# fxcawley/nanoSandbox

Hardware: AMD Instinct MI355X
Metric: tokens/sec (whole node) GPT-2 124M DDP (higher is better)
Workload: dtype bf16

## Files before the change

csrc/kernels/gemm_wg4.hip:

```cpp
#include <utility>

#include "common.h"

namespace {

constexpr int W_BM = 256, W_BN = 256, W_BK = 64;
constexpr int W_THR = 256;
constexpr int W_IMG = W_BK * 256 * 2;
constexpr int W_SMEM = 4 * W_IMG;
constexpr int W_GRP = 3072;

enum : int { W_EPI_ATOMIC = 1, W_EPI_STORE = 4 };

typedef int w_i32x4 __attribute__((ext_vector_type(4)));

struct Wg4Args {
  const bf16_t* A;
  const bf16_t* B;
  float* C;
  float* gb;
  int M, N, K;
  int lda, ldb, ldc;
  int tiles_m, tiles_n, splits;
};

template <int I>
struct WI {
  static constexpr int value = I;
};
template <class F, int... Is>
__device__ __forceinline__ void w_for_impl(F&& f, std::integer_sequence<int, Is...>) {
  (f(WI<Is>{}), ...);
}
template <int N, class F>
__device__ __forceinline__ void w_for(F&& f) {
  w_for_impl(f, std::make_integer_sequence<int, N>{});
}

template <bool H>
__device__ __forceinline__ void w_mfma(f32x4& acc, const bf16x8& b, const bf16x8& a) {
  if constexpr (H) asm volatile("v_mfma_f32_16x16x32_f16 %0, %1, %2, %0" : "+a"(acc) : "v"(b), "v"(a));
  else asm volatile("v_mfma_f32_16x16x32_bf16 %0, %1, %2, %0" : "+a"(acc) : "v"(b), "v"(a));
}
// ... 14 lines not shown
}
template <int OFF>
__device__ __forceinline__ void w_dma(uint32_t lds, uint32_t voff, w_i32x4 rsrc, uint32_t soff) {
  if constexpr (OFF == 0) {
    asm volatile("s_mov_b32 m0, %0\n\ts_nop 0\n\tbuffer_load_dwordx4 %1, %2, %3 offen lds" ::"s"(lds), "v"(voff),
                 "s"(rsrc), "s"(soff)
                 : "memory");
  } else {
    asm volatile("buffer_load_dwordx4 %0, %1, %2 offen offset:%3 lds" ::"v"(voff), "s"(rsrc), "s"(soff), "n"(OFF)
                 : "memory");
  }
}
#ifndef NSA_WG4_GLDS
#define NSA_WG4_GLDS 0
#endif
template <int OFF>
__device__ __forceinline__ void w_dmag(uint32_t lds, uint32_t voff, const void* sbase) {
  if constexpr (OFF == 0) {
    asm volatile("s_mov_b32 m0, %0\n\ts_nop 0\n\tglobal_load_lds_dwordx4 %1, %2" ::"s"(lds), "v"(voff), "s"(sbase)
                 : "memory");
  } else {
    asm volatile("global_load_lds_dwordx4 %0, %1 offset:%2" ::"v"(voff), "s"(sbase), "n"(OFF) : "memory");
  }
}
__device__ __forceinline__ w_i32x4 w_rsrc(const void* base, uint32_t bytes) {
  const uint64_t b = (uint64_t)(uintptr_t)base;
  w_i32x4 r;
  r.x = __builtin_amdgcn_readfirstlane((int)(uint32_t)b);
  r.y = __builtin_amdgcn_readfirstlane((int)(uint32_t)(b >> 32) & 0xffff);
  r.z = __builtin_amdgcn_readfirstlane((int)bytes);
  r.w = 0x00020000;
  return r;
}
__device__ __forceinline__ void w_add_base(w_i32x4& r, uint32_t bytes) {
  uint64_t b = ((uint64_t)(uint32_t)r.y << 32) | (uint32_t)r.x;
  b += bytes;
  r.x = (int)(uint32_t)b;
  r.y = (int)(uint32_t)(b >> 32);
}
__device__ __forceinline__ s16x4 w_tr(uint32_t addr) {
  return __builtin_amdgcn_ds_read_tr16_b64_v4i16((__attribute__((address_space(3))) s16x4*)(uintptr_t)addr);
}
__device__ __forceinline__ bf16x8 w_cat(s16x4 a, s16x4 b) {
  typedef short s16x8 __attribute__((ext_vector_type(8)));
  s16x8 v = __builtin_shufflevector(a, b, 0, 1, 2, 3, 4, 5, 6, 7);
  return __builtin_bit_cast(bf16x8, v);
// ... 93 lines not shown
      w_dmag<(p & 3) * 1024>(dmaA + buf + (uint32_t)((p & 4) * 1024), vpA[p], sbase(ra));
    else
      w_dma<(p & 3) * 1024>(dmaA + buf + (uint32_t)((p & 4) * 1024), voA[(p & 1) | ((p >> 2) << 1)], ra, soA[p]);
  };
  auto issue_b = [&](uint32_t buf, auto P) {
    constexpr int p = decltype(P)::value;
    if constexpr (NSA_WG4_GLDS)
      w_dmag<(p & 3) * 1024>(dmaB + buf + (uint32_t)((p & 4) * 1024), vpB[p], sbase(rb));
    else
      w_dma<(p & 3) * 1024>(dmaB + buf + (uint32_t)((p & 4) * 1024), voB[(p & 1) | ((p >> 2) << 1)], rb, soB[p]);
  };

  const int ig = lane & 15, fq = ig >> 2, fp = ig & 3;
  const int krow = 8 * (lane >> 4) + fq;
  const int gk = w_g(krow);
  uint32_t rdA[8], rdB[8];
#pragma unroll
  for (int f = 0; f < 8; ++f) {
    const int fa = wm * 8 + f, fb = wn * 8 + f;
    rdA[f] = lds0 + (uint32_t)(krow * 512 + (((2 * fa + (fp >> 1)) ^ (2 * gk)) << 4) + (fp & 1) * 8);
    rdB[f] = lds0 + (uint32_t)(2 * W_IMG + krow * 512 + (((2 * fb + (fp >> 1)) ^ (2 * gk)) << 4) + (fp & 1) * 8);
  }

  w_for<8>([&](auto P) { issue_a(0, P); });
  w_for<8>([&](auto P) { issue_b(0, P); });
  cur_next();
  w_for<8>([&](auto P) { issue_a(W_IMG, P); });
  w_for<8>([&](auto P) { issue_b(W_IMG, P); });
  w_vmwait<16>();
  cur_next();
  w_barrier();

  f32x4 acc[8][8];
  bf16x8 a0[8], b0[8], a1[8], b1[8];
#pragma unroll
  for (int f = 0; f < 8; ++f) {
    a0[f] = w_cat(w_tr(rdA[f]), w_tr(rdA[f] + 2048));
    b0[f] = w_cat(w_tr(rdB[f]), w_tr(rdB[f] + 2048));
  }

  float bsum[8] = {0.f, 0.f, 0.f, 0.f, 0.f, 0.f, 0.f, 0.f};
  int kc = kt0;
  uint32_t buf = 0;
  auto ktile = [&](auto FIRST_) {
    constexpr bool FIRST = decltype(FIRST_)::value;
    const bool do_bg = BG && kc % g.tiles_n == tn;
    w_for<128>([&](auto I) {
      constexpr int n = decltype(I)::value;
      constexpr int kk = n >> 6, j = (n >> 3) & 7, i = n & 7;
      if constexpr (kk == 0) {
        if constexpr (FIRST) w_mfma0<H>(acc[i][j], b0[j], a0[i]);
        else w_mfma<H>(acc[i][j], b0[j], a0[i]);
      } else {
        w_mfma<H>(acc[i][j], b1[j], a1[i]);
      }
      if constexpr (BG && j == 1) {
// ... 14 lines not shown
        constexpr int pc = (n - D0) / DS;
        if constexpr (pc < 8) issue_a(buf, WI<pc>{});
        else issue_b(buf, WI<pc - 8>{});
      }
      if constexpr (n == 62) {
#pragma unroll
        for (int f = 0; f < 8; ++f) {
          rdA[f] ^= (uint32_t)W_IMG;
          rdB[f] ^= (uint32_t)W_IMG;
        }
      }
      if constexpr (n == 92) w_vmwait<(92 - D0) / DS + 1>();
      if constexpr (n == 93) w_barrier();
      if constexpr (n >= 94 && n < 126 && ((n - 94) & 1) == 0) {
        constexpr int f = ((n - 94) >> 1) & 7;
        if constexpr (n < 110) b0[f] = w_cat(w_tr(rdB[f]), w_tr(rdB[f] + 2048));
        else a0[f] = w_cat(w_tr(rdA[f]), w_tr(rdA[f] + 2048));
      }
    });
    buf ^= (uint32_t)W_IMG;
    cur_next();
    ++kc;
  };
  ktile(WI<1>{});
  for (int kt = 1; kt < nk; ++kt) ktile(WI<0>{});
  asm volatile("s_waitcnt vmcnt(0) lgkmcnt(0)\n\ts_nop 7\n\ts_nop 7\n\ts_nop 7" ::: "memory");
  if constexpr (BG) {
    const int first = kt0 + ((tn - kt0 % g.tiles_n) + g.tiles_n) % g.tiles_n;
    if (first < kt1) {
#pragma unroll
      for (int f = 0; f < 8; ++f) {
        if ((f & 1) != wn) continue;
        float v = bsum[f];
        v += __shfl_xor(v, 16);
        v += __shfl_xor(v, 32);
        const int m = m0 + wm * 128 + 16 * f + (lane & 15);
        if (lane < 16 && m >= mlo) atomicAdd(g.gb + m, v);
      }
    }
  }
  w_barrier();

  char* ep = smem + wave * 32768;
  const int er = lane & 15, eq = lane >> 4;
  float* Cz = g.C;
  if constexpr (EPI == W_EPI_STORE) Cz += (int64_t)z * g.M * g.ldc;
#pragma unroll
  for (int half = 0; half < 2; ++half) {
#pragma unroll
    for (int ii = 0; ii < 4; ++ii) {
      const int i = 4 * half + ii;
      const int row = 16 * ii + er;
#pragma unroll
      for (int j = 0; j < 8; ++j) {
        const int u = 4 * j + eq;
        *reinterpret_cast<f32x4*>(ep + row * 512 + ((u ^ (row & 7)) << 4)) = acc[i][j];
      }
    }
    __builtin_amdgcn_fence(__ATOMIC_SEQ_CST, "wavefront");
    __builtin_amdgcn_wave_barrier();
    const int col0 = n0 + wn * 128;
    const int rot = (z * 23) & 63;
#pragma unroll 4
    for (int r2 = 0; r2 < 64; ++r2) {
      const int rr = (r2 + rot) & 63;
      const int grow = m0 + wm * 128 + 64 * half + rr;
#pragma unroll
      for (int c2 = 0; c2 < 2; ++c2) {
        const int c = 64 * c2 + lane;
        const float val = *reinterpret_cast<const float*>(ep + rr * 512 + ((((c >> 2) ^ (rr & 7))) << 4) + (c & 3) * 4);
        if (grow >= mlo && col0 + c >= nlo) {
          if constexpr (EPI == W_EPI_STORE)
            Cz[(int64_t)grow * g.ldc + col0 + c] = val;
          else
            atomicAdd(Cz + (int64_t)grow * g.ldc + col0 + c, val);
        }
      }
    }
    __builtin_amdgcn_fence(__ATOMIC_SEQ_CST, "wavefront");
    __builtin_amdgcn_wave_barrier();
  }
}

namespace {
template <bool H>
hipError_t wgrad4_entry(int epi, const void* A, int lda, const void* B, int ldb, void* C, int ldc, void* gb, int M,
                        int N, int K, int splits, hipStream_t s) {
  if (gb && epi != W_EPI_ATOMIC) return hipErrorInvalidValue;
  if ((epi != W_EPI_ATOMIC && epi != W_EPI_STORE) || M < W_BM || N < W_BN || M % 8 || N % 8 || K % W_BK ||
      splits < 1 || splits > K / W_BK || lda % 8 || ldb % 8 || lda < M || ldb < N || ldc < N)
    return hipErrorInvalidValue;
  if ((int64_t)W_BK * lda * 2 + W_GRP >= (1ll << 31) || (int64_t)W_BK * ldb * 2 + W_GRP >= (1ll << 31))
    return hipErrorInvalidValue;
  Wg4Args a{};
  a.A = (const bf16_t*)A;
  a.B = (const bf16_t*)B;
  a.C = (float*)C;
  a.M = M;
  a.N = N;
  a.K = K;
  a.lda = lda;
  a.ldb = ldb;
  a.ldc = ldc;
  a.tiles_m = (M + W_BM - 1) / W_BM;
  a.tiles_n = (N + W_BN - 1) / W_BN;
  a.splits = splits;
  const dim3 grid(a.tiles_m * a.tiles_n * splits);
  a.gb = (float*)gb;
  if (gb) wgrad4_kernel<W_EPI_ATOMIC, true, H><<<grid, W_THR, 0, s>>>(a);
  else if (epi == W_EPI_ATOMIC) wgrad4_kernel<W_EPI_ATOMIC, false, H><<<grid, W_THR, 0, s>>>(a);
  else wgrad4_kernel<W_EPI_STORE, false, H><<<grid, W_THR, 0, s>>>(a);
  return hipGetLastError();
}
}

NSA_API hipError_t nsa_gemm_wgrad4b(int epi, const void* A, int lda, const void* B, int ldb, void* C, int ldc, void* gb,
                                    int M, int N, int K, int splits, hipStream_t s) {
  return wgrad4_entry<false>(epi, A, lda, B, ldb, C, ldc, gb, M, N, K, splits, s);
}
NSA_API hipError_t nsa_gemm_wgrad4(int epi, const void* A, int lda, const void* B, int ldb, void* C, int ldc, int M,
                                   int N, int K, int splits, hipStream_t s) {
  return wgrad4_entry<false>(epi, A, lda, B, ldb, C, ldc, nullptr, M, N, K, splits, s);
}
NSA_API hipError_t nsa_gemm_wgrad4b_h(int epi, const void* A, int lda, const void* B, int ldb, void* C, int ldc,
                                      void* gb, int M, int N, int K, int splits, hipStream_t s) {
  return wgrad4_entry<true>(epi, A, lda, B, ldb, C, ldc, gb, M, N, K, splits, s);
}
NSA_API hipError_t nsa_gemm_wgrad4_h(int epi, const void* A, int lda, const void* B, int ldb, void* C, int ldc, int M,
                                     int N, int K, int splits, hipStream_t s) {
  return wgrad4_entry<true>(epi, A, lda, B, ldb, C, ldc, nullptr, M, N, K, splits, s);
}
```

nanosandbox_amd/ops/_lib.py:

```python

from __future__ import annotations

import ctypes
import os
import threading

import torch

_LIB_DIR = os.path.join(os.path.dirname(os.path.dirname(os.path.abspath(__file__))), "lib")
LIB_PATH = os.environ.get("NSA_KERNEL_LIB") or os.path.join(_LIB_DIR, "libnsa_kernels.so")

_lock = threading.Lock()
_lib = None

c_void_p = ctypes.c_void_p
c_int = ctypes.c_int
c_int64 = ctypes.c_int64
c_uint64 = ctypes.c_uint64
c_float = ctypes.c_float

_SIGNATURES = {
    "nsa_embedding_fwd": [c_void_p, c_void_p, c_void_p, c_void_p, c_int, c_int, c_int, c_float, c_uint64, c_void_p],
    "nsa_embedding_bwd": [c_void_p, c_void_p, c_void_p, c_void_p, c_int, c_int, c_int, c_float, c_uint64, c_void_p],
    "nsa_embedding_fwd_x32": [c_void_p, c_void_p, c_void_p, c_void_p, c_int, c_int, c_int, c_float, c_uint64,
# ... 55 lines not shown
                           c_void_p],
    "nsa_skinny_ln_gemm_q8": [c_void_p, c_void_p, c_void_p, c_void_p, c_void_p, c_float, c_void_p, c_void_p,
                              c_void_p, c_void_p, c_int, c_int, c_int, c_int, c_int, c_void_p],
    "nsa_gemv_emb_ln_q8": [c_void_p, c_void_p, c_void_p, c_void_p, c_void_p, c_void_p, c_void_p, c_void_p, c_void_p,
                           c_void_p, c_void_p, c_int, c_int, c_float, c_int, c_int, c_void_p],
    "nsa_gemv_attn_q8": [c_void_p, c_int, c_void_p, c_void_p, c_void_p, c_void_p, c_int, c_int, c_int, c_int,
                         c_void_p],
    "nsa_gemv_ln_q8": [c_void_p, c_void_p, c_void_p, c_void_p, c_void_p, c_void_p, c_void_p, c_void_p, c_void_p,
                       c_int, c_int, c_float, c_int, c_int, c_void_p, c_void_p],
    "nsa_flash_bwd2": [c_void_p, c_void_p, c_void_p, c_void_p, c_void_p, c_void_p,
                       c_int, c_int, c_int, c_int, c_float, c_float, c_uint64, c_void_p],
    "nsa_rng_advance": [c_void_p],
    "nsa_rng_set": [c_uint64, c_void_p],
    "nsa_splitk_reduce": [c_void_p, c_void_p, c_int64, c_int, c_void_p],
    "nsa_embedding_bwd_det": [c_void_p, c_void_p, c_void_p, c_void_p, c_void_p, c_void_p, c_void_p, c_int, c_int,
                              c_int, c_int, c_int, c_float, c_uint64, c_void_p],
    "nsa_transpose_bf16": [c_void_p, c_void_p, c_int, c_int, c_void_p],
    "nsa_gemm": [c_int, c_int, c_void_p, c_int, c_void_p, c_int, c_void_p, c_int, c_void_p, c_void_p,
                 c_int, c_int, c_int, c_int, c_void_p],
    "nsa_gemm_wgrad4": [c_int, c_void_p, c_int, c_void_p, c_int, c_void_p, c_int, c_int, c_int, c_int, c_int,
                        c_void_p],
    "nsa_gemm_wgrad4b": [c_int, c_void_p, c_int, c_void_p, c_int, c_void_p, c_int, c_void_p, c_int, c_int, c_int, c_int,
                         c_void_p],
    "nsa_gemm_nt4": [c_int, c_void_p, c_int, c_void_p, c_int, c_void_p, c_int, c_void_p, c_void_p, c_void_p,
                     c_int, c_int, c_int, c_int, c_void_p],
    "nsa_gemm_small": [c_int, c_void_p, c_int, c_void_p, c_int, c_void_p, c_int, c_void_p, c_void_p, c_void_p,
                       c_int, c_int, c_int, c_void_p],
    "nsa_gemm_nt4_xent": [c_void_p, c_int, c_void_p, c_int, c_void_p, c_int, c_void_p, c_void_p, c_int, c_int, c_int,
                          c_int, c_int, c_void_p],
    "nsa_gemm_nt4_xdx": [c_void_p, c_int, c_void_p, c_int, c_void_p, c_int, c_void_p, c_void_p, c_int, c_int, c_int,
                         c_int, c_void_p],
    "nsa_xent_tlogit": [c_void_p, c_int, c_void_p, c_int, c_void_p, c_void_p, c_void_p, c_int, c_int, c_int, c_float,
                        c_void_p],
    "nsa_xent_combine": [c_void_p, c_int, c_void_p, c_void_p, c_void_p, c_void_p, c_void_p, c_int, c_float, c_float,
                         c_float, c_void_p],
    "nsa_xent_fixup": [c_void_p, c_int, c_void_p, c_int, c_void_p, c_int, c_void_p, c_void_p, c_void_p, c_void_p,
                       c_void_p, c_int, c_int, c_int, c_void_p],
    "nsa_xent_bwd_prep": [c_void_p, c_int, c_void_p, c_int, c_void_p, c_void_p, c_void_p, c_void_p, c_void_p,
                          c_void_p, c_int, c_int, c_void_p],
    "nsa_xent_dw_fix": [c_void_p, c_int, c_void_p, c_int, c_void_p, c_void_p, c_void_p, c_void_p, c_int, c_int, c_int,
                        c_void_p],
    "nsa_xent_dw_fix_sorted": [c_void_p, c_int, c_void_p, c_int, c_void_p, c_void_p, c_void_p, c_void_p, c_void_p,
                               c_void_p, c_void_p, c_void_p, c_int, c_int, c_int, c_int, c_void_p],
    "nsa_embedding_bwd_lds": [c_void_p, c_void_p, c_void_p, c_void_p, c_void_p, c_int, c_int, c_int, c_int, c_int,
                              c_float, c_uint64, c_void_p],
    "nsa_seg_lds_parts": [c_int],
    "nsa_xent_dw_fix_lds": [c_void_p, c_int, c_void_p, c_int, c_void_p, c_void_p, c_void_p, c_void_p, c_void_p,
                            c_int, c_int, c_int, c_int, c_void_p],
    "nsa_colsum_bf16_partial": [c_void_p, c_int, c_int, c_int, c_void_p, c_int, c_void_p],
    "nsa_keysort": [c_void_p, c_int, c_int, c_int, c_void_p, c_void_p, c_void_p, c_void_p, c_void_p],
    "nsa_keysort_ws_bytes": [c_int],
    "nsa_probe_spin": [c_int, c_uint64, c_void_p, c_void_p],
    "nsa_probe_mark": [c_void_p, c_void_p],
}
_RESTYPES = {"nsa_keysort_ws_bytes": c_int64}


class KernelLibraryMissing(RuntimeError):
    pass


def lib():
    global _lib
    if _lib is not None:
        return _lib
    with _lock:
        if _lib is not None:
            return _lib
        if not os.path.exists(LIB_PATH):
            raise KernelLibraryMissing(
                f"HIP kernel library not found at {LIB_PATH}; build it with "
                "`python -m nanosandbox_amd.build` (hipcc --offload-arch=gfx950)")
        L = ctypes.CDLL(LIB_PATH, mode=ctypes.RTLD_GLOBAL)
        for name, argtypes in _SIGNATURES.items():
            for sym in (name, name + "_h"):
                fn = getattr(L, sym, None)
                if fn is None:
                    continue
# ... 33 lines not shown
```

nanosandbox_amd/ops/gemm.py:

```python

from __future__ import annotations

import os

import torch

from . import _lib

BF16 = torch.bfloat16
F16 = torch.float16
LAYOUT_TN = 2


def _sym(name, t):
    if t.dtype == F16:
        return name + "_h"
    if t.dtype != BF16:
        raise ValueError(f"GEMM kernels take bf16 or fp16 operands, got {t.dtype}")
    return name
EPI_ATOMIC, EPI_STORE_F32 = 1, 4
BK = 64
TILE = 256


def _check(t, name):
# ... 199 lines not shown
                      _lib.ptr(g32), K_in, _lib.ptr(gb32), N_out, K_in, T, splits, _lib.stream())
            return g32
        wgrad_acc(dy2, x2, g32, splits, deterministic)
        bias_grad_acc(dy2, gb32, deterministic)
        return g32

    def launch(epi, C):
        if four:
            _lib.call(_sym("nsa_gemm_wgrad4", dy2), epi, _lib.ptr(dy2), dy2.stride(0), _lib.ptr(x2), x2.stride(0), _lib.ptr(C),
                      K_in, N_out, K_in, T, splits, _lib.stream())
        else:
            _lib.call(_sym("nsa_gemm", dy2), LAYOUT_TN, epi, _lib.ptr(dy2), dy2.stride(0), _lib.ptr(x2), x2.stride(0),
                      _lib.ptr(C), K_in, None, None, N_out, K_in, T, splits, _lib.stream())

    if deterministic and splits > 1:
        ws = torch.empty(splits, N_out, K_in, device=g32.device, dtype=torch.float32)
        launch(EPI_STORE_F32, ws)
        _lib.call("nsa_splitk_reduce", _lib.ptr(ws), _lib.ptr(g32), g32.numel(), splits, _lib.stream())
        return g32
    launch(EPI_ATOMIC, g32)
    return g32


def bias_grad_acc(dy2, gb32, deterministic=False):
    T, N = dy2.shape
    _check(dy2, "dy")
    nblk = max(1, min(256, T // 64))
    part = torch.empty(nblk, N, device=dy2.device, dtype=torch.float32)
    _lib.call(_sym("nsa_colsum_bf16_partial", dy2), _lib.ptr(dy2), dy2.stride(0), T, N, _lib.ptr(part), nblk, _lib.stream())
    _lib.call("nsa_colsum_accum_ordered" if deterministic else "nsa_colsum_accum", _lib.ptr(part), _lib.ptr(gb32),
              nblk, N, _lib.stream())
    return gb32
```

nanosandbox_amd/ops/gemm_dispatch.py:

```python

from __future__ import annotations

import os

import torch

from . import _lib
from . import gemm as _gemm

F32 = torch.float32
BF16 = torch.bfloat16

DETERMINISTIC = False


F16 = torch.float16



def _ok(*ts):
    return (ts[0].dtype in (BF16, F16)
            and all(t.is_cuda and t.dtype == ts[0].dtype and t.is_contiguous() and t.data_ptr() % 16 == 0
                    for t in ts))


def kernel_for(op: str, M: int, N: int, K: int) -> str:
# ... 41 lines not shown


def _gelu_grad_torch(uf):
    cdf = 0.5 * (1.0 + torch.erf(uf * 0.7071067811865476))
    return cdf + uf * torch.exp(-0.5 * uf * uf) * 0.3989422804014327


def fwd(x2, w, b=None):
    return _nt(x2, w, bias=b)


def fwd_gelu(x2, w, b=None):
    return _nt(x2, w, epi=_gemm.NT_EPI_GELU, bias=b, op="fwd_gelu")


def dgrad(dy2, w):
    return _nt(dy2, _wt(w), op="dgrad")


def dgrad_dgelu(dy2, w, gp):
    return _nt(dy2, _wt(w), epi=_gemm.NT_EPI_DGELU, u=gp, op="dgrad_dgelu")


def wgrad_acc(dy2, x2, g32, gb32=None):
    T, N = dy2.shape
    K = x2.shape[1]
    k = kernel_for("wgrad", N, K, T) if _ok(dy2, x2) and g32.is_contiguous() else "torch"
    _used.setdefault(("wgrad", N, K, T), k if k == "torch" else f"{k}/s{_gemm.wgrad_splits(N, K, T)}")
    if k != "torch":
        if gb32 is not None and not (gb32.is_contiguous() and dy2.shape[1] % 8 == 0):
            _gemm.wgrad_acc(dy2, x2, g32, deterministic=DETERMINISTIC)
            bias_grad_acc(dy2, gb32)
            return
        _gemm.wgrad_acc(dy2, x2, g32, deterministic=DETERMINISTIC, gb32=gb32)
        return
    g32.add_(dy2.t().float() @ x2.float())
    if gb32 is not None:
        gb32.add_(dy2.float().sum(0))


def bias_grad_acc(dy2, gb32):
    if _ok(dy2) and dy2.shape[1] % 8 == 0 and gb32.is_contiguous():
        _gemm.bias_grad_acc(dy2, gb32, deterministic=DETERMINISTIC)
        return
    gb32.add_(dy2.float().sum(0))


_weight_gen = 0


def weights_changed():
# ... 28 lines not shown
```

nanosandbox_amd/optim/flat.py:

```python

from __future__ import annotations

from dataclasses import dataclass

import torch

CHUNK = 64


@dataclass
class ParamSlot:
    name: str
    param: torch.nn.Parameter
    offset: int
    numel: int
    padded: int
    decay: bool


class FlatParamStore:
    def __init__(self, model: torch.nn.Module, device, compute_dtype=None, fused_grad=True):
        self.device = torch.device(device)
        named = [(n, p) for n, p in model.named_parameters() if p.requires_grad]
        self.slots: list[ParamSlot] = []
        off = 0
        for name, p in reversed(named):
            n = p.numel()
            rows = getattr(p, "_nsa_pad_rows", None)
            room = rows * p.shape[1] if rows and p.dim() == 2 and rows > p.shape[0] else n
            padded = (room + CHUNK - 1) // CHUNK * CHUNK
            self.slots.append(ParamSlot(name, p, off, n, padded, p.dim() >= 2))
            off += padded
        self.numel = off
        self.master = torch.zeros(off, dtype=torch.float32, device=self.device)
        self.grad = torch.zeros(off, dtype=torch.float32, device=self.device)
        flags = torch.zeros(off // CHUNK, dtype=torch.uint8)
        with torch.no_grad():
            for s in self.slots:
                view = self.master[s.offset:s.offset + s.numel]
                view.copy_(s.param.detach().reshape(-1).to(self.device, torch.float32))
                s.param.data = view.view(s.param.shape)
                if s.decay:
                    flags[s.offset // CHUNK:(s.offset + s.padded) // CHUNK] = 1
        self.wd_mask = flags.to(self.device)
        self.fused_grad = fused_grad
        for s in self.slots:
            g = self.grad[s.offset:s.offset + s.numel].view(s.param.shape)
            if fused_grad:
                s.param.main_grad = g
                pr = self._pad_shape(s)
                if pr is not None:
                    s.param.main_grad_padded = self.grad[s.offset:s.offset + pr[0] * pr[1]].view(pr)
            else:
                s.param.grad = g
        self.compute_dtype = compute_dtype
        self.compute = None
        if compute_dtype is not None and compute_dtype != torch.float32:
            self.compute = torch.empty(off, dtype=compute_dtype, device=self.device)
            for s in self.slots:
                s.param.compute = self.compute[s.offset:s.offset + s.numel].view(s.param.shape)
                pr = self._pad_shape(s)
                if pr is not None:
                    s.param.compute_padded = self.compute[s.offset:s.offset + pr[0] * pr[1]].view(pr)
            self.refresh_compute()

    @staticmethod
    def _pad_shape(s: ParamSlot):
        rows = getattr(s.param, "_nsa_pad_rows", None)
# ... 4 lines not shown
    def slot_of(self, p) -> ParamSlot:
        for s in self.slots:
            if s.param is p:
                return s
        raise KeyError("parameter not in store")

    def param_view(self, buf: torch.Tensor, s: ParamSlot) -> torch.Tensor:
        return buf[s.offset:s.offset + s.numel].view(s.param.shape)

    @torch.no_grad()
    def refresh_compute(self):
        from ..ops import gemm_dispatch
        gemm_dispatch.weights_changed()
        if self.compute is None:
            return
        if self.device.type == "cuda":
            from ..ops import _lib
            name = "nsa_cast_f32_bf16_h" if self.compute.dtype == torch.float16 else "nsa_cast_f32_bf16"
            _lib.call(name, _lib.ptr(self.master), _lib.ptr(self.compute), self.numel, _lib.stream())
        else:
            self.compute.copy_(self.master)

    @torch.no_grad()
    def zero_grad(self):
        self.grad.zero_()
        if not self.fused_grad:
            for s in self.slots:
                if s.param.grad is None or s.param.grad.data_ptr() != self.param_view(self.grad, s).data_ptr():
                    s.param.grad = self.param_view(self.grad, s)

    def buckets(self, cap_bytes: int):
        out = []
        start = 0
        size = 0
        members = []
        late = False
        for s in self.slots:
            nbytes = s.padded * 4
            is_late = bool(getattr(s.param, "_nsa_late_grad", False))
            if members and (is_late != late or (size + nbytes > cap_bytes and not is_late)):
                out.append((start, s.offset, members))
                start = s.offset
                size = 0
                members = []
            members.append(s)
            size += nbytes
            late = is_late
        if members:
# ... 3 lines not shown
```

nanosandbox_amd/runtime/hipgraph.py:

```python

from __future__ import annotations

import torch


def graph_capture_supported(device: str, dropout: float, world_size: int, ddp_impl: str = "flat",
                            gas: int = 2) -> tuple[bool, str]:
    if not str(device).startswith("cuda") or not torch.cuda.is_available():
        return False, "graph capture needs a GPU device"
    if world_size > 1 and ddp_impl != "flat":
        return False, "torch DDP: its reducer hooks autograd (use ddp_impl='flat')"
    if world_size > 1 and gas < 2:
        return False, "one micro-step per rank: the synchronising micro-step always runs eagerly"
    return True, ""


class MicroStepGraph:

    def __init__(self, model, X: torch.Tensor, Y: torch.Tensor, gas: int, warmup: int = 2, zero_grad=None,
                 dropout: bool = False, loss_scale: torch.Tensor | None = None):
        from ..ops import rng_advance

        self.model = model
        self.gas = gas
        self.X = X.detach().clone()
        self.Y = Y.detach().clone()
        side = torch.cuda.Stream()
        side.wait_stream(torch.cuda.current_stream())
        with torch.cuda.stream(side):
            for _ in range(warmup):
                if dropout:
                    rng_advance(self.X.device)
                _, loss = model(self.X, self.Y)
                ((loss / gas) * loss_scale if loss_scale is not None else loss / gas).backward()
        torch.cuda.current_stream().wait_stream(side)
        torch.cuda.synchronize()
        if zero_grad is not None:
            zero_grad()
        self.graph = torch.cuda.CUDAGraph()
        with torch.cuda.graph(self.graph):
            if dropout:
                rng_advance(self.X.device)
            _, loss = model(self.X, self.Y)
            self.loss = loss / gas
            (self.loss * loss_scale if loss_scale is not None else self.loss).backward()
        self.replays = 0

    def run(self, X: torch.Tensor, Y: torch.Tensor) -> torch.Tensor:
        self.X.copy_(X, non_blocking=True)
        self.Y.copy_(Y, non_blocking=True)
        self.graph.replay()
        self.replays += 1
        return self.loss
```

nanosandbox_amd/train.py:

```python

from __future__ import annotations

import os
import sys
import time

import torch

from .config import TRAIN_DEFAULTS, config_keys, parse_argv
from .data import load_meta, make_batch_source, resolve_data_dir
from .ops import rng_advance
from .ops.functional import XENT_F16_GUARD as xent_f16_guard
from .runtime import MicroStepGraph, graph_capture_supported
from .models import GPT, GPTConfig
from .optim import FlatParamStore
from .parallel import FlatBucketReducer, destroy, init_distributed
from .utils import MetricsLogger, get_lr, load_checkpoint, load_model_state, save_checkpoint


_DTYPES = {"bfloat16": torch.bfloat16, "float16": torch.float16, "float32": torch.float32}


def _compute_dtype(device_type: str, dtype: str) -> torch.dtype:
    if dtype not in _DTYPES:
        raise ValueError(f"dtype must be one of {sorted(_DTYPES)}, got {dtype!r}")
    if device_type != "cuda":
        return torch.float32
    return _DTYPES[dtype]


class Trainer:
    def __init__(self, cfg: dict):
        self.cfg = cfg
        c = cfg
        self.info = init_distributed(c["backend"], c["device"])
# ... 79 lines not shown
        fused_grad = self.ddp_impl != "torch"
        shadow = self.compute_dtype if self.compute_dtype in (torch.bfloat16, torch.float16) else None
        self.store = FlatParamStore(model, self.device, compute_dtype=shadow if self.device_type == "cuda" else None,
                                    fused_grad=fused_grad)
        self.optimizer = model.configure_optimizers(c["weight_decay"], c["learning_rate"], (c["beta1"], c["beta2"]),
                                                    self.device_type, store=self.store)
        if self.scaler is not None:
            self.optimizer.attach_loss_scale(self.scaler)
        if init_from == "resume" and checkpoint is not None:
            self.optimizer.load_state_dict(checkpoint["optimizer"])
        checkpoint = None
        self.activation_plan = None
        if self.device_type == "cuda" and (c["grad_ckpt"] or c["hbm_plan"]):
            from .utils.memory import plan_grad_ckpt
            free, _ = torch.cuda.mem_get_info(torch.device(self.device))
            self.activation_plan = plan_grad_ckpt(
                model.config.n_layer, model.config.n_embd, model.config.n_head, model.config.vocab_size,
                c["batch_size"] * c["block_size"], free, fp32_residual=c["fp32_residual"], requested=c["grad_ckpt"],
                recompute_mlp=c["recompute_mlp"])
            model.grad_ckpt = self.activation_plan.grad_ckpt
            model.recompute_mlp = self.activation_plan.recompute_mlp
            if self.master:
                print(self.activation_plan.describe())
        self.graph = None
        self.use_graph = False
        if c["compile"]:
            ok, why = graph_capture_supported(self.device, c["dropout"], info.world_size, self.ddp_impl, self.gas)
            if ok and self.compute_dtype not in (torch.bfloat16, torch.float16):
                ok, why = False, f"dtype={c['dtype']} runs the torch reference ops"
            self.use_graph = ok
            if self.master:
                print(("compile=True: micro-step captured as a HIP graph" +
                       (" (the synchronising micro-step runs eagerly)" if info.world_size > 1 else "")) if ok
                      else f"compile=True: eager micro-steps ({why})")

        self.raw_model = model
        self.model = model
        self.reducer = None
        if info.ddp:
            if self.ddp_impl == "flat":
                rdt = torch.bfloat16 if c["grad_reduce_dtype"] == "bfloat16" else torch.float32
                self.reducer = FlatBucketReducer(self.store, bucket_cap_mb=c["ddp_bucket_mb"], reduce_dtype=rdt)
                self.reducer.broadcast_parameters()
                self.optimizer.grad_scale = self.reducer.grad_scale
                if self.master:
                    print(f"DDP: flat bucketed reducer, {len(self.reducer.buckets)} buckets "
                          f"(cap {c['ddp_bucket_mb']} MiB, {c['grad_reduce_dtype']})")
            elif self.ddp_impl == "torch":
                from torch.nn.parallel import DistributedDataParallel as DDP
                dev_ids = [torch.device(self.device).index] if self.device_type == "cuda" else None
                self.model = DDP(model, device_ids=dev_ids, bucket_cap_mb=c["ddp_bucket_mb"])
                self.store.refresh_compute()
            else:
                raise ValueError(f"unknown ddp_impl {self.ddp_impl!r}")

        if info.ddp and c["rccl_report"]:
            from .parallel import report_transport
            self.rccl_report = report_transport(info)

        self._grad_scale0 = self.optimizer.grad_scale
        self.batches = make_batch_source(c["dataset"], c["data_dir"], c["block_size"], c["batch_size"], self.device,
                                         seed=c["seed"] + info.seed_offset, vocab_size=model_args["vocab_size"])
        run_name = c["wandb_run_name"] or "run"
        self.metrics = MetricsLogger(c["out_dir"], jsonl=c["metrics_jsonl"], tensorboard_dir=c["tensorboard_dir"],
                                     run_name=run_name, enabled=self.master)
        if c["wandb_log"] and self.master:
            print("wandb_log=True: wandb is not installed in this image; logging to metrics.jsonl/tfevents instead")

    @torch.no_grad()
    def estimate_loss(self):
        out = {}
        m = self.raw_model
        m.eval()
        for split in ["train", "val"]:
            losses = torch.zeros(self.cfg["eval_iters"], device=self.device)
            for k in range(self.cfg["eval_iters"]):
                X, Y = self.batches.get_batch(split)
                _, loss = m(X, Y)
                losses[k] = loss.float()
            out[split] = losses.mean().item()
        m.train()
        return out

    def _save(self):
        print(f"saving checkpoint to {self.cfg['out_dir']}")
        save_checkpoint(os.path.join(self.cfg["out_dir"], "ckpt.pt"), self.raw_model, self.optimizer,
                        self.model_args, self.iter_num, self.best_val_loss,
                        {k: self.cfg[k] for k in config_keys(self.cfg)})

    def train_step(self, X, Y):
        c = self.cfg
        n_graph = (self.gas - 1 if self.reducer is not None else self.gas) if self.use_graph else 0
        if n_graph > 0:
            if self.graph is None:
                if self.reducer is not None:
                    self.reducer.prepare(False)
                self.graph = MicroStepGraph(self.model, X, Y, self.gas,
                                            zero_grad=lambda: self.optimizer.zero_grad(set_to_none=True),
                                            dropout=c["dropout"] > 0.0,
                                            loss_scale=self.scaler.scale_t if self.scaler is not None else None)
            for _ in range(n_graph):
                loss = self.graph.run(X, Y)
                X, Y = self.batches.get_batch("train")
        for micro_step in range(n_graph, self.gas):
            sync = micro_step == self.gas - 1
            if self.reducer is not None:
                self.reducer.prepare(sync)
            elif self.ddp_impl == "torch":
                self.model.require_backward_grad_sync = sync
            if c["dropout"] > 0.0:
                rng_advance(self.device)
            _, loss = self.model(X, Y)
            loss = loss / self.gas
            X, Y = self.batches.get_batch("train")
            (loss * self.scaler.scale_t if self.scaler is not None else loss).backward()
        if self.reducer is not None:
            self.reducer.finish()
        norm = None
        if c["grad_clip"] != 0.0:
            norm = self.optimizer.clip_grad_norm_(c["grad_clip"])
        self.optimizer.step()
        if norm is None and self.scaler is not None and hasattr(self.optimizer, "last_norm"):
            norm = self.optimizer.last_norm
        self.optimizer.zero_grad(set_to_none=True)
        if self.scaler is not None and xent_f16_guard.poll():
            self.graph = None
        return loss, norm, X, Y

    def fit(self):
        c = self.cfg
        X, Y = self.batches.get_batch("train")
        t0 = time.time()
        local_iter_num = 0
        running_mfu = -1.0
        prof = self._profiler() if c["profile"] and self.master else None
        while True:
            lr = get_lr(self.iter_num, c["learning_rate"], c["warmup_iters"], c["lr_decay_iters"], c["min_lr"]) \
                if c["decay_lr"] else c["learning_rate"]
            for param_group in self.optimizer.param_groups:
                param_group["lr"] = lr
# ... 87 lines not shown
```

nanosandbox_amd/utils/memory.py:

```python

from __future__ import annotations

from dataclasses import dataclass

GiB = 1 << 30


@dataclass
class ActivationPlan:
    tokens: int
    resident_bytes: int
    ckpt_bytes: int
    budget_bytes: int
    grad_ckpt: bool
    reason: str
    recompute_mlp: bool = False
    mlp_recompute_bytes: int = 0

    def describe(self) -> str:
        return (f"activation plan: {self.tokens} tokens/micro-step, resident {self.resident_bytes / GiB:.1f} GiB, "
                f"MLP-recompute {self.mlp_recompute_bytes / GiB:.1f} GiB, checkpointed {self.ckpt_bytes / GiB:.1f} "
                f"GiB, budget {self.budget_bytes / GiB:.1f} GiB -> grad_ckpt={self.grad_ckpt} "
                f"recompute_mlp={self.recompute_mlp} ({self.reason})")

# ... 29 lines not shown
    budget = int(headroom * free_bytes)

    def plan(gc, rm, why):
        return ActivationPlan(tokens, res, ck, budget, gc, why, recompute_mlp=rm, mlp_recompute_bytes=sel)
    if requested:
        return plan(True, False, "requested by config")
    if recompute_mlp:
        return plan(False, True, "MLP recompute requested by config")
    if free_bytes <= 0:
        return plan(False, False, "free memory unknown")
    if res <= budget:
        return plan(False, False, "fits resident")
    if sel <= budget:
        return plan(False, True, "resident estimate exceeds the budget; MLP recompute fits")
    return plan(True, False, "resident and MLP-recompute estimates exceed the budget" +
                ("" if ck <= budget else "; checkpointed may not fit either"))


def model_state_bytes(n_layer: int, n_embd: int, vocab_size: int, block_size: int) -> int:
    n_params = 12 * n_layer * n_embd * n_embd + (vocab_size + block_size) * n_embd
    return 20 * n_params


RUNTIME_RESERVE = 8 * GiB


def choose_micro_batch(n_layer: int, n_embd: int, n_head: int, vocab_size: int, block_size: int,
                       per_rank_seqs: int, hbm_bytes: int, fp32_residual: bool = True, cap: int = 120,
                       headroom: float = 0.9) -> tuple[int, bool]:
    budget = headroom * (hbm_bytes - model_state_bytes(n_layer, n_embd, vocab_size, block_size) - RUNTIME_RESERVE)
    divisors = [d for d in range(min(cap, per_rank_seqs), 0, -1) if per_rank_seqs % d == 0]
    kw = dict(n_layer=n_layer, n_embd=n_embd, n_head=n_head, vocab_size=vocab_size, fp32_residual=fp32_residual)
    for d in divisors:
        if activation_bytes(tokens=d * block_size, **kw) <= budget:
            return d, False
    for d in divisors:
        if activation_bytes(tokens=d * block_size, grad_ckpt=True, **kw) <= budget:
            return d, True
    return divisors[-1], True
```

Measured before the change: 1.235 million.

## Accumulate split-K weight gradients in private slots instead of atomics

Adds a private-slot epilogue to the four-wave weight-gradient GEMM. Each split-K block loads its earlier partial accumulator from a dedicated fp32 slot, continues the MFMA accumulation across micro-steps, and stores it back with nontemporal vector stores, replacing the LDS-staged atomicAdd epilogue. A separate reduce kernel sums the splits into the fp32 gradient once per sync step, driven by a device-side table and flag. This is meant to remove atomic contention and the LDS round trip, at the cost of a large extra workspace, slot load/store traffic on every micro-step, and a reduction pass.

```diff
diff --git a/csrc/kernels/gemm_wg4.hip b/csrc/kernels/gemm_wg4.hip
--- a/csrc/kernels/gemm_wg4.hip
+++ b/csrc/kernels/gemm_wg4.hip
@@ -1,6 +1,11 @@
 #include <utility>
 
 #include "common.h"
+#include "wg4_slot.h"
+
+#ifndef NSA_WG4_PROBE_NOEPI
+#define NSA_WG4_PROBE_NOEPI 0
+#endif
 
 namespace {
 
@@ -10,7 +15,7 @@
 constexpr int W_SMEM = 4 * W_IMG;
 constexpr int W_GRP = 3072;
 
-enum : int { W_EPI_ATOMIC = 1, W_EPI_STORE = 4 };
+enum : int { W_EPI_ATOMIC = 1, W_EPI_STORE = 4, W_EPI_PRIVATE = 8 };
 
 typedef int w_i32x4 __attribute__((ext_vector_type(4)));
 
@@ -19,6 +24,7 @@
   const bf16_t* B;
   float* C;
   float* gb;
+  const int* flag;
   int M, N, K;
   int lda, ldb, ldc;
   int tiles_m, tiles_n, splits;
@@ -79,6 +85,17 @@
   } else {
     asm volatile("global_load_lds_dwordx4 %0, %1 offset:%2" ::"v"(voff), "s"(sbase), "n"(OFF) : "memory");
   }
+}
+template <int OFF>
+__device__ __forceinline__ void w_slot_ld(f32x4& acc, uint32_t voff, w_i32x4 rsrc, uint32_t soff) {
+  asm volatile("buffer_load_dwordx4 %0, %1, %2, %3 offen offset:%4 nt"
+               : "=a"(acc)
+               : "v"(voff), "s"(rsrc), "s"(soff), "n"(OFF)
+               : "memory");
+}
+template <int OFF>
+__device__ __forceinline__ void w_slot_st(const f32x4& acc, uint32_t voff, const void* sbase) {
+  asm volatile("global_store_dwordx4 %0, %1, %2 offset:%3 nt" ::"v"(voff), "a"(acc), "s"(sbase), "n"(OFF) : "memory");
 }
 __device__ __forceinline__ w_i32x4 w_rsrc(const void* base, uint32_t bytes) {
   const uint64_t b = (uint64_t)(uintptr_t)base;
@@ -218,6 +235,23 @@
     rdB[f] = lds0 + (uint32_t)(2 * W_IMG + krow * 512 + (((2 * fb + (fp >> 1)) ^ (2 * gk)) << 4) + (fp & 1) * 8);
   }
 
+  f32x4 acc[8][8];
+  const void* slot_base = nullptr;
+  const uint32_t slot_vo = (uint32_t)(lane * 16 + 4096);
+  if constexpr (EPI == W_EPI_PRIVATE) {
+    static_assert(!BG, "the bias gradient stays on atomics");
+    const uint64_t sb = (uint64_t)(uintptr_t)(reinterpret_cast<const f32x4*>(g.C) + (int64_t)u * WG4_SLOT_VEC +
+                                              wg4_slot_vec(wave, 0, 0, 0));
+    slot_base = reinterpret_cast<const void*>(
+        ((uint64_t)(uint32_t)__builtin_amdgcn_readfirstlane((int)(uint32_t)(sb >> 32)) << 32) |
+        (uint32_t)__builtin_amdgcn_readfirstlane((int)(uint32_t)sb));
+    const w_i32x4 rs = w_rsrc(slot_base, *g.flag != 0 ? (uint32_t)(WG4_WAVE_VEC * 16) : 0u);
+    w_for<64>([&](auto I) {
+      constexpr int n = decltype(I)::value;
+      w_slot_ld<(n & 3) * 1024>(acc[n >> 3][n & 7], (uint32_t)(lane * 16), rs, (uint32_t)((n >> 2) * 4096));
+    });
+  }
+
   w_for<8>([&](auto P) { issue_a(0, P); });
   w_for<8>([&](auto P) { issue_b(0, P); });
   cur_next();
@@ -227,7 +261,6 @@
   cur_next();
   w_barrier();
 
-  f32x4 acc[8][8];
   bf16x8 a0[8], b0[8], a1[8], b1[8];
 #pragma unroll
   for (int f = 0; f < 8; ++f) {
@@ -288,7 +321,8 @@
     cur_next();
     ++kc;
   };
-  ktile(WI<1>{});
+  if constexpr (EPI == W_EPI_PRIVATE) ktile(WI<0>{});
+  else ktile(WI<1>{});
   for (int kt = 1; kt < nk; ++kt) ktile(WI<0>{});
   asm volatile("s_waitcnt vmcnt(0) lgkmcnt(0)\n\ts_nop 7\n\ts_nop 7\n\ts_nop 7" ::: "memory");
   if constexpr (BG) {
@@ -304,6 +338,14 @@
         if (lane < 16 && m >= mlo) atomicAdd(g.gb + m, v);
       }
     }
+  }
+  if constexpr (NSA_WG4_PROBE_NOEPI == 2) return;
+  if constexpr (EPI == W_EPI_PRIVATE) {
+    w_for<64>([&](auto I) {
+      constexpr int n = decltype(I)::value;
+      w_slot_st<(n & 7) * 1024 - 4096>(acc[n >> 3][n & 7], slot_vo + (uint32_t)((n >> 3) * 8192), slot_base);
+    });
+    return;
   }
   w_barrier();
 
@@ -335,7 +377,7 @@
       for (int c2 = 0; c2 < 2; ++c2) {
         const int c = 64 * c2 + lane;
         const float val = *reinterpret_cast<const float*>(ep + rr * 512 + ((((c >> 2) ^ (rr & 7))) << 4) + (c & 3) * 4);
-        if (grow >= mlo && col0 + c >= nlo) {
+        if (NSA_WG4_PROBE_NOEPI == 0 && grow >= mlo && col0 + c >= nlo) {
           if constexpr (EPI == W_EPI_STORE)
             Cz[(int64_t)grow * g.ldc + col0 + c] = val;
           else
@@ -378,6 +420,83 @@
   else wgrad4_kernel<W_EPI_STORE, false, H><<<grid, W_THR, 0, s>>>(a);
   return hipGetLastError();
 }
+
+template <bool H>
+hipError_t wgrad4p_entry(const void* A, int lda, const void* B, int ldb, void* slots, const void* flag, int M, int N,
+                         int K, int splits, hipStream_t s) {
+  if (!slots || !flag || ((uintptr_t)slots & 15) || M < W_BM || N < W_BN || M % 8 || N % 8 || K % W_BK || splits < 1 ||
+      splits > K / W_BK || lda % 8 || ldb % 8 || lda < M || ldb < N)
+    return hipErrorInvalidValue;
+  if ((int64_t)W_BK * lda * 2 + W_GRP >= (1ll << 31) || (int64_t)W_BK * ldb * 2 + W_GRP >= (1ll << 31))
+    return hipErrorInvalidValue;
+  Wg4Args a{};
+  a.A = (const bf16_t*)A;
+  a.B = (const bf16_t*)B;
+  a.C = (float*)slots;
+  a.flag = (const int*)flag;
+  a.M = M;
+  a.N = N;
+  a.K = K;
+  a.lda = lda;
+  a.ldb = ldb;
+  a.tiles_m = (M + W_BM - 1) / W_BM;
+  a.tiles_n = (N + W_BN - 1) / W_BN;
+  a.splits = splits;
+  wgrad4_kernel<W_EPI_PRIVATE, false, H><<<dim3(a.tiles_m * a.tiles_n * splits), W_THR, 0, s>>>(a);
+  return hipGetLastError();
+}
+
+__global__ __launch_bounds__(W_THR) void wg4_reduce_kernel(const Wg4ReduceEntry* __restrict__ tab, int n, int base,
+                                                                const int* __restrict__ flag) {
+  if (flag && *flag == 0) return;
+  const int b = base + blockIdx.x;
+  int e = 0;
+  while (e + 1 < n && tab[e + 1].block0 <= b) ++e;
+  const Wg4ReduceEntry w = tab[e];
+  const int v = b - w.block0;
+  if (v >= w.tiles) return;
+  const int tm = v / w.tiles_n, tn = v % w.tiles_n;
+  const int mlo = tm * W_BM, nlo = tn * W_BN;
+  const int m0 = min(mlo, w.M - W_BM), n0 = min(nlo, w.N - W_BN);
+  const int lane = threadIdx.x & 63, wave = threadIdx.x >> 6;
+  const f32x4* slot = reinterpret_cast<const f32x4*>(w.slots) + (int64_t)v * WG4_SLOT_VEC;
+  const int64_t zstride = (int64_t)w.tiles * WG4_SLOT_VEC;
+  {
+    const int i = blockIdx.y;
+    const int row = m0 + wg4_frag_row(wave, lane, i);
+    if (row < mlo) return;
+    f32x4 sum[8];
+#pragma unroll
+    for (int j = 0; j < 8; ++j) sum[j] = __builtin_nontemporal_load(slot + wg4_slot_vec(wave, lane, i, j));
+    for (int z = 1; z < w.splits; ++z) {
+#pragma unroll
+      for (int j = 0; j < 8; ++j)
+        sum[j] += __builtin_nontemporal_load(slot + z * zstride + wg4_slot_vec(wave, lane, i, j));
+    }
+#pragma unroll
+    for (int j = 0; j < 8; ++j) {
+      const int col = n0 + wg4_frag_col(wave, lane, j);
+      if (col < nlo) continue;
+      f32x4* p = reinterpret_cast<f32x4*>(w.grad + (int64_t)row * w.ldc + col);
+      *p += sum[j];
+    }
+  }
+}
+}
+
+NSA_API hipError_t nsa_wgrad4_reduce(const void* table, int n, int base, int blocks, const void* flag, hipStream_t s) {
+  if (!table || n < 1 || base < 0 || blocks < 1) return hipErrorInvalidValue;
+  wg4_reduce_kernel<<<dim3(blocks, 8), W_THR, 0, s>>>((const Wg4ReduceEntry*)table, n, base, (const int*)flag);
+  return hipGetLastError();
+}
+NSA_API int nsa_wgrad4_reduce_entry_bytes() { return (int)sizeof(Wg4ReduceEntry); }
+NSA_API hipError_t nsa_gemm_wgrad4p(const void* A, int lda, const void* B, int ldb, void* slots, const void* flag,
+                                    int M, int N, int K, int splits, hipStream_t s) {
+  return wgrad4p_entry<false>(A, lda, B, ldb, slots, flag, M, N, K, splits, s);
+}
+NSA_API hipError_t nsa_gemm_wgrad4p_h(const void* A, int lda, const void* B, int ldb, void* slots, const void* flag,
+                                      int M, int N, int K, int splits, hipStream_t s) {
+  return wgrad4p_entry<true>(A, lda, B, ldb, slots, flag, M, N, K, splits, s);
 }
 
 NSA_API hipError_t nsa_gemm_wgrad4b(int epi, const void* A, int lda, const void* B, int ldb, void* C, int ldc, void* gb,
diff --git a/csrc/kernels/wg4_slot.h b/csrc/kernels/wg4_slot.h
--- /dev/null
+++ b/csrc/kernels/wg4_slot.h
@@ -0,0 +1,24 @@
+#pragma once
+
+constexpr int WG4_TILE = 256;
+constexpr int WG4_SLOT_VEC = WG4_TILE * WG4_TILE / 4;
+constexpr int WG4_WAVE_VEC = 64 * 64;
+
+__host__ __device__ constexpr int wg4_slot_vec(int wave, int lane, int i, int j) {
+  return wave * WG4_WAVE_VEC + (8 * i + j) * 64 + lane;
+}
+__host__ __device__ constexpr int wg4_frag_row(int wave, int lane, int i) {
+  return (wave >> 1) * 128 + 16 * i + (lane & 15);
+}
+__host__ __device__ constexpr int wg4_frag_col(int wave, int lane, int j) {
+  return (wave & 1) * 128 + 16 * j + 4 * (lane >> 4);
+}
+
+struct Wg4ReduceEntry {
+  float* grad;
+  const float* slots;
+  int ldc, M, N;
+  int tiles_n, tiles, splits;
+  int block0;
+  int pad;
+};
diff --git a/nanosandbox_amd/ops/_lib.py b/nanosandbox_amd/ops/_lib.py
--- a/nanosandbox_amd/ops/_lib.py
+++ b/nanosandbox_amd/ops/_lib.py
@@ -101,6 +101,9 @@
                         c_void_p],
     "nsa_gemm_wgrad4b": [c_int, c_void_p, c_int, c_void_p, c_int, c_void_p, c_int, c_void_p, c_int, c_int, c_int, c_int,
                          c_void_p],
+    "nsa_gemm_wgrad4p": [c_void_p, c_int, c_void_p, c_int, c_void_p, c_void_p, c_int, c_int, c_int, c_int, c_void_p],
+    "nsa_wgrad4_reduce": [c_void_p, c_int, c_int, c_int, c_void_p, c_void_p],
+    "nsa_wgrad4_reduce_entry_bytes": [],
     "nsa_gemm_nt4": [c_int, c_void_p, c_int, c_void_p, c_int, c_void_p, c_int, c_void_p, c_void_p, c_void_p,
                      c_int, c_int, c_int, c_int, c_void_p],
     "nsa_gemm_small": [c_int, c_void_p, c_int, c_void_p, c_int, c_void_p, c_int, c_void_p, c_void_p, c_void_p,
@@ -132,7 +135,7 @@
     "nsa_probe_spin": [c_int, c_uint64, c_void_p, c_void_p],
     "nsa_probe_mark": [c_void_p, c_void_p],
 }
-_RESTYPES = {"nsa_keysort_ws_bytes": c_int64}
+_RESTYPES = {"nsa_keysort_ws_bytes": c_int64, "nsa_wgrad4_reduce_entry_bytes": c_int}
 
 
 class KernelLibraryMissing(RuntimeError):
diff --git a/nanosandbox_amd/ops/gemm.py b/nanosandbox_amd/ops/gemm.py
--- a/nanosandbox_amd/ops/gemm.py
+++ b/nanosandbox_amd/ops/gemm.py
@@ -1,6 +1,7 @@
 
 from __future__ import annotations
 
+import ctypes
 import os
 
 import torch
@@ -246,6 +247,67 @@
     return g32
 
 
+SLOT_FLOATS = TILE * TILE
+
+
+def wgrad_tiles(n_out, n_in) -> int:
+    return -(-n_out // TILE) * -(-n_in // TILE)
+
+
+def wgrad_private(dy2, x2, slots, flag, splits):
+    T, N_out = dy2.shape
+    K_in = x2.shape[1]
+    _check(dy2, "dy")
+    _check(x2, "x")
+    if not wgrad4_supported(N_out, K_in, T):
+        raise ValueError(f"no private weight-gradient kernel for [{N_out}, {K_in}] over {T} tokens")
+    need = wgrad_tiles(N_out, K_in) * splits * SLOT_FLOATS
+    if slots.dtype != torch.float32 or not slots.is_contiguous() or slots.numel() < need:
+        raise ValueError(f"slots must be a contiguous fp32 tensor of at least {need} elements")
+    if flag.dtype != torch.int32 or flag.numel() != 1:
+        raise ValueError("flag must be one int32 on the device")
+    _lib.call(_sym("nsa_gemm_wgrad4p", dy2), _lib.ptr(dy2), dy2.stride(0), _lib.ptr(x2), x2.stride(0), _lib.ptr(slots),
+              _lib.ptr(flag), N_out, K_in, T, splits, _lib.stream())
+
+
+class _ReduceEntry(ctypes.Structure):
+    _fields_ = [("grad", ctypes.c_void_p), ("slots", ctypes.c_void_p), ("ldc", ctypes.c_int), ("M", ctypes.c_int),
+                ("N", ctypes.c_int), ("tiles_n", ctypes.c_int), ("tiles", ctypes.c_int), ("splits", ctypes.c_int),
+                ("block0", ctypes.c_int), ("pad", ctypes.c_int)]
+
+
+def wgrad_reduce_table(weights, device):
+    if _lib.call_ret("nsa_wgrad4_reduce_entry_bytes") != ctypes.sizeof(_ReduceEntry):
+        raise RuntimeError("Wg4ReduceEntry layout differs from the kernel library's")
+    arr = (_ReduceEntry * len(weights))()
+    spans = []
+    b0 = 0
+    for e, (g32, slots, splits) in zip(arr, weights):
+        M, N = g32.shape
+        if (g32.dtype != torch.float32 or g32.stride(1) != 1 or g32.stride(0) % 4 or g32.data_ptr() % 16
+                or M < TILE or N < TILE or N % 4 or slots.data_ptr() % 16):
+            raise ValueError("gradient rows must be fp32, 16-byte aligned, on a four-wave shape")
+        tiles = wgrad_tiles(M, N)
+        if slots.numel() < tiles * splits * SLOT_FLOATS:
+            raise ValueError("slots too small")
+        e.grad, e.slots, e.ldc, e.M, e.N = g32.data_ptr(), slots.data_ptr(), g32.stride(0), M, N
+        e.tiles_n, e.tiles, e.splits, e.block0 = -(-N // TILE), tiles, splits, b0
+        spans.append((b0, tiles))
+        b0 += tiles
+    host = torch.frombuffer(bytearray(bytes(arr)), dtype=torch.uint8)
+    return host.to(device), spans
+
+
+def wgrad_reduce(table, spans, which=None, flag=None):
+    esz = ctypes.sizeof(_ReduceEntry)
+    if which is None:
+        _lib.call("nsa_wgrad4_reduce", _lib.ptr(table), len(spans), 0, spans[-1][0] + spans[-1][1], _lib.ptr(flag),
+                  _lib.stream())
+    else:
+        b0, n = spans[which]
+        _lib.call("nsa_wgrad4_reduce", table.data_ptr() + which * esz, 1, b0, n, _lib.ptr(flag), _lib.stream())
+
+
 def bias_grad_acc(dy2, gb32, deterministic=False):
     T, N = dy2.shape
     _check(dy2, "dy")
diff --git a/nanosandbox_amd/ops/gemm_dispatch.py b/nanosandbox_amd/ops/gemm_dispatch.py
--- a/nanosandbox_amd/ops/gemm_dispatch.py
+++ b/nanosandbox_amd/ops/gemm_dispatch.py
@@ -2,6 +2,7 @@
 from __future__ import annotations
 
 import os
+import weakref
 
 import torch
 
@@ -89,11 +90,33 @@
     return _nt(dy2, _wt(w), epi=_gemm.NT_EPI_DGELU, u=gp, op="dgrad_dgelu")
 
 
+_wgrad_ws = None
+
+
+def set_wgrad_workspace(ws) -> None:
+    global _wgrad_ws
+    _wgrad_ws = None if ws is None else weakref.ref(ws)
+
+
+def wgrad_workspace():
+    return None if _wgrad_ws is None else _wgrad_ws()
+
+
+def wgrad_micro_step_done() -> None:
+    ws = wgrad_workspace()
+    if ws is not None:
+        ws.micro_step_done()
+
+
 def wgrad_acc(dy2, x2, g32, gb32=None):
     T, N = dy2.shape
     K = x2.shape[1]
     k = kernel_for("wgrad", N, K, T) if _ok(dy2, x2) and g32.is_contiguous() else "torch"
     _used.setdefault(("wgrad", N, K, T), k if k == "torch" else f"{k}/s{_gemm.wgrad_splits(N, K, T)}")
+    if k == "wgrad4" and gb32 is None and not DETERMINISTIC:
+        ws = wgrad_workspace()
+        if ws is not None and ws.launch(dy2, x2, g32):
+            return
     if k != "torch":
         if gb32 is not None and not (gb32.is_contiguous() and dy2.shape[1] % 8 == 0):
             _gemm.wgrad_acc(dy2, x2, g32, deterministic=DETERMINISTIC)
diff --git a/nanosandbox_amd/ops/wgrad_private.py b/nanosandbox_amd/ops/wgrad_private.py
--- /dev/null
+++ b/nanosandbox_amd/ops/wgrad_private.py
@@ -0,0 +1,113 @@
+
+from __future__ import annotations
+
+import os
+import weakref
+from dataclasses import dataclass
+
+import torch
+
+from . import gemm as _gemm
+
+SLOT_BYTES = _gemm.SLOT_FLOATS * 4
+
+
+def enabled() -> bool:
+    return os.environ.get("NSA_WGRAD_PRIVATE", "1") != "0"
+
+
+@dataclass
+class SlotSpan:
+    name: str
+    n_out: int
+    n_in: int
+    tokens: int
+    splits: int
+    tiles: int
+    slot0: int
+
+    @property
+    def slots(self) -> int:
+        return self.splits * self.tiles
+
+
+def layout(weights, tokens: int) -> list[SlotSpan]:
+    out, s0 = [], 0
+    for name, n_out, n_in in weights:
+        if not _gemm.wgrad4_supported(n_out, n_in, tokens):
+            continue
+        sp = SlotSpan(name, n_out, n_in, tokens, _gemm.wgrad_splits(n_out, n_in, tokens),
+                      _gemm.wgrad_tiles(n_out, n_in), s0)
+        out.append(sp)
+        s0 += sp.slots
+    return out
+
+
+def layout_bytes(spans) -> int:
+    return sum(sp.slots for sp in spans) * SLOT_BYTES
+
+
+def gpt_weights(n_layer: int, n_embd: int, vocab_rows: int, bias: bool = False):
+    C = n_embd
+    w = [("lm_head", vocab_rows, C)]
+    if not bias:
+        for i in range(n_layer):
+            w += [(f"h.{i}.attn.c_attn", 3 * C, C), (f"h.{i}.attn.c_proj", C, C), (f"h.{i}.mlp.c_fc", 4 * C, C),
+                  (f"h.{i}.mlp.c_proj", C, 4 * C)]
+    return w
+
+
+class WgradWorkspace:
+    def __init__(self, grads, tokens: int, device):
+        self.device = torch.device(device)
+        self.tokens = tokens
+        elig = [(n, g) for n, g in grads if g.dim() == 2 and g.is_contiguous() and g.data_ptr() % 16 == 0
+                and g.shape[1] % 4 == 0]
+        self.spans = layout([(n, g.shape[0], g.shape[1]) for n, g in elig], tokens)
+        byname = dict(elig)
+        grads = [byname[sp.name] for sp in self.spans]
+        self.nbytes = layout_bytes(self.spans)
+        self.ws = torch.zeros(self.nbytes // 4, device=self.device, dtype=torch.float32)
+        self.flag = torch.zeros(1, device=self.device, dtype=torch.int32)
+        self._index = {id(g): (i, weakref.ref(g)) for i, g in enumerate(grads)}
+        self.table, self.blocks = (None, [])
+        if self.spans:
+            self.table, self.blocks = _gemm.wgrad_reduce_table(
+                [(g, self.slots_of(i), sp.splits) for i, (g, sp) in enumerate(zip(grads, self.spans))],
+                self.device)
+        self.reduce_each = False
+        self._launched = set()
+
+    def slots_of(self, i: int) -> torch.Tensor:
+        sp = self.spans[i]
+        return self.ws[sp.slot0 * _gemm.SLOT_FLOATS:(sp.slot0 + sp.slots) * _gemm.SLOT_FLOATS]
+
+    def launch(self, dy2, x2, g32) -> bool:
+        hit = self._index.get(id(g32))
+        if hit is None or hit[1]() is not g32:
+            return False
+        i = hit[0]
+        sp = self.spans[i]
+        if (dy2.shape[0], dy2.shape[1], x2.shape[1]) != (sp.tokens, sp.n_out, sp.n_in) or i in self._launched:
+            return False
+        self._launched.add(i)
+        _gemm.wgrad_private(dy2, x2, self.slots_of(i), self.flag, sp.splits)
+        if self.reduce_each:
+            _gemm.wgrad_reduce(self.table, self.blocks, which=i)
+        return True
+
+    def micro_step_done(self):
+        if self.reduce_each:
+            self.flag.zero_()
+        else:
+            self.flag.fill_(1)
+        self._launched.clear()
+
+    def reduce_all(self):
+        if self.spans:
+            _gemm.wgrad_reduce(self.table, self.blocks, flag=self.flag)
+        self.clear()
+
+    def clear(self):
+        self.flag.zero_()
+        self._launched.clear()
diff --git a/nanosandbox_amd/optim/flat.py b/nanosandbox_amd/optim/flat.py
--- a/nanosandbox_amd/optim/flat.py
+++ b/nanosandbox_amd/optim/flat.py
@@ -44,6 +44,7 @@
                     flags[s.offset // CHUNK:(s.offset + s.padded) // CHUNK] = 1
         self.wd_mask = flags.to(self.device)
         self.fused_grad = fused_grad
+        self.wgrad_ws = None
         for s in self.slots:
             g = self.grad[s.offset:s.offset + s.numel].view(s.param.shape)
             if fused_grad:
@@ -94,8 +95,15 @@
             self.compute.copy_(self.master)
 
     @torch.no_grad()
+    def finalize_grad(self):
+        if self.wgrad_ws is not None:
+            self.wgrad_ws.reduce_all()
+
+    @torch.no_grad()
     def zero_grad(self):
         self.grad.zero_()
+        if self.wgrad_ws is not None:
+            self.wgrad_ws.clear()
         if not self.fused_grad:
             for s in self.slots:
                 if s.param.grad is None or s.param.grad.data_ptr() != self.param_view(self.grad, s).data_ptr():
diff --git a/nanosandbox_amd/runtime/hipgraph.py b/nanosandbox_amd/runtime/hipgraph.py
--- a/nanosandbox_amd/runtime/hipgraph.py
+++ b/nanosandbox_amd/runtime/hipgraph.py
@@ -20,6 +20,7 @@
     def __init__(self, model, X: torch.Tensor, Y: torch.Tensor, gas: int, warmup: int = 2, zero_grad=None,
                  dropout: bool = False, loss_scale: torch.Tensor | None = None):
         from ..ops import rng_advance
+        from ..ops.gemm_dispatch import wgrad_micro_step_done
 
         self.model = model
         self.gas = gas
@@ -33,6 +34,7 @@
                     rng_advance(self.X.device)
                 _, loss = model(self.X, self.Y)
                 ((loss / gas) * loss_scale if loss_scale is not None else loss / gas).backward()
+                wgrad_micro_step_done()
         torch.cuda.current_stream().wait_stream(side)
         torch.cuda.synchronize()
         if zero_grad is not None:
@@ -44,6 +46,7 @@
             _, loss = model(self.X, self.Y)
             self.loss = loss / gas
             (self.loss * loss_scale if loss_scale is not None else self.loss).backward()
+            wgrad_micro_step_done()
         self.replays = 0
 
     def run(self, X: torch.Tensor, Y: torch.Tensor) -> torch.Tensor:
diff --git a/nanosandbox_amd/train.py b/nanosandbox_amd/train.py
--- a/nanosandbox_amd/train.py
+++ b/nanosandbox_amd/train.py
@@ -11,6 +11,7 @@
 from .data import load_meta, make_batch_source, resolve_data_dir
 from .ops import rng_advance
 from .ops.functional import XENT_F16_GUARD as xent_f16_guard
+from .ops.gemm_dispatch import wgrad_micro_step_done
 from .runtime import MicroStepGraph, graph_capture_supported
 from .models import GPT, GPTConfig
 from .optim import FlatParamStore
@@ -136,6 +137,7 @@
             model.recompute_mlp = self.activation_plan.recompute_mlp
             if self.master:
                 print(self.activation_plan.describe())
+        self.wgrad_ws = self._make_wgrad_workspace(model)
         self.graph = None
         self.use_graph = False
         if c["compile"]:
@@ -181,6 +183,47 @@
         if c["wandb_log"] and self.master:
             print("wandb_log=True: wandb is not installed in this image; logging to metrics.jsonl/tfevents instead")
 
+    def _make_wgrad_workspace(self, model):
+        from .ops import gemm_dispatch, wgrad_private
+        gemm_dispatch.set_wgrad_workspace(None)
+        c = self.cfg
+        if (self.device_type != "cuda" or not self.store.fused_grad or c["deterministic"]
+                or self.compute_dtype not in (torch.bfloat16, torch.float16) or not wgrad_private.enabled()):
+            return None
+        grads = []
+        for name, m in model.named_modules():
+            if isinstance(m, torch.nn.Linear) and m.bias is None and m.weight.requires_grad:
+                g = getattr(m.weight, "main_grad_padded", None)
+                g = getattr(m.weight, "main_grad", None) if g is None else g
+                if g is not None:
+                    grads.append((name, g))
+        tokens = c["batch_size"] * c["block_size"]
+        nbytes = wgrad_private.layout_bytes(wgrad_private.layout([(n, g.shape[0], g.shape[1]) for n, g in grads
+                                                                   if g.dim() == 2], tokens))
+        if nbytes == 0:
+            return None
+        free, _ = torch.cuda.mem_get_info(torch.device(self.device))
+        if self.activation_plan is not None:
+            from .utils.memory import wgrad_workspace_keeps_plan
+            cfgm = model.config
+            fits = wgrad_workspace_keeps_plan(
+                nbytes, free, n_layer=cfgm.n_layer, n_embd=cfgm.n_embd, n_head=cfgm.n_head, vocab_size=cfgm.vocab_size,
+                tokens=tokens, fp32_residual=c["fp32_residual"], requested=c["grad_ckpt"],
+                recompute_mlp=c["recompute_mlp"])
+        else:
+            fits = nbytes < 0.25 * free
+        if not fits:
+            if self.master:
+                print(f"weight gradients: atomic epilogue (the {nbytes / 2 ** 30:.1f} GiB of private split-K slots "
+                      "would change the activation plan)")
+            return None
+        ws = wgrad_private.WgradWorkspace(grads, tokens, self.device)
+        self.store.wgrad_ws = ws
+        gemm_dispatch.set_wgrad_workspace(ws)
+        if self.master:
+            print(f"weight gradients: private split-K slots, {len(ws.spans)} weights, {ws.nbytes / 2 ** 30:.2f} GiB")
+        return ws
+
     @torch.no_grad()
     def estimate_loss(self):
         out = {}
@@ -220,6 +263,8 @@
             sync = micro_step == self.gas - 1
             if self.reducer is not None:
                 self.reducer.prepare(sync)
+                if self.wgrad_ws is not None:
+                    self.wgrad_ws.reduce_each = sync
             elif self.ddp_impl == "torch":
                 self.model.require_backward_grad_sync = sync
             if c["dropout"] > 0.0:
@@ -228,8 +273,12 @@
             loss = loss / self.gas
             X, Y = self.batches.get_batch("train")
             (loss * self.scaler.scale_t if self.scaler is not None else loss).backward()
+            wgrad_micro_step_done()
         if self.reducer is not None:
             self.reducer.finish()
+            if self.wgrad_ws is not None:
+                self.wgrad_ws.reduce_each = False
+        self.store.finalize_grad()
         norm = None
         if c["grad_clip"] != 0.0:
             norm = self.optimizer.clip_grad_norm_(c["grad_clip"])
diff --git a/nanosandbox_amd/utils/memory.py b/nanosandbox_amd/utils/memory.py
--- a/nanosandbox_amd/utils/memory.py
+++ b/nanosandbox_amd/utils/memory.py
@@ -75,6 +75,22 @@
     return 20 * n_params
 
 
+def wgrad_workspace_bytes(n_layer: int, n_embd: int, vocab_size: int, tokens: int, bias: bool = False) -> int:
+    from ..ops import lm_head_rows
+    from ..ops import wgrad_private as wp
+    return wp.layout_bytes(wp.layout(wp.gpt_weights(n_layer, n_embd, lm_head_rows(vocab_size), bias), tokens))
+
+
+def wgrad_workspace_keeps_plan(ws_bytes: int, free_bytes: int, **plan_kw) -> bool:
+    if free_bytes <= 0:
+        return True
+    if ws_bytes >= free_bytes:
+        return False
+    a = plan_grad_ckpt(free_bytes=free_bytes, **plan_kw)
+    b = plan_grad_ckpt(free_bytes=free_bytes - ws_bytes, **plan_kw)
+    return (a.grad_ckpt, a.recompute_mlp) == (b.grad_ckpt, b.recompute_mlp)
+
+
 RUNTIME_RESERVE = 8 * GiB
 
 
```

Result: no change. 1.240 million (median of 6 runs) (+0.3%).
